# KTH-RPL/cloth-splatting

Hardware: AMD Instinct MI355X
Metric: rasterizer fwd+bwd rendered Mpix/s (scene_1, 800x800) (higher is better)
Workload: dtype f32

## Files before the change

cloth-splatting_amd/csrc/csplat_raster.hip:

```cpp
#include "csplat_common.h"

#include <atomic>
#include <cstring>
#include <chrono>
#include <mutex>
#include <type_traits>

#include "csplat_raster_math.h"
#include "csplat_raster_k1.h"
#include "csplat_raster_binning.h"
#include "csplat_raster_k5b_k6.h"

namespace {

constexpr int ACC_STRIDE = 16;

#define CSPLAT_ROWMASK_OP(OP, dst, src0, src1, RM)                                                                                  \
    asm("s_nop 1\n\tv_" OP "_f32_dpp %0, %1, %2 quad_perm:[0,1,2,3] row_mask:" RM " bank_mask:0xf" : "+v"(dst) : "v"(src0), "v"(src1))
__device__ __forceinline__ void rows_scan_mul(float f, float Tin, float &Tr, float &Tout) {
    const auto s16 = __builtin_amdgcn_permlane16_swap(__float_as_uint(f), __float_as_uint(f), false, false);
    const float ev = __uint_as_float(s16[0]), od = __uint_as_float(s16[1]);
    const float pr = ev * od;
    const auto s32 = __builtin_amdgcn_permlane32_swap(__float_as_uint(pr), __float_as_uint(pr), false, false);
    const float lo = __uint_as_float(s32[0]), hi = __uint_as_float(s32[1]);
// ... 613 lines not shown
    return (g_stamp_buf && g_stamp_words == 8u * ((size_t)cdiv(P, 64) + (size_t)cdiv(P, 32))) ? g_stamp_buf : nullptr;
}

int tsort_mode(int P) { return (P < (1 << 24) ? 1 : 0) | (dbg(CSPLAT_DEBUG_SORT_RADIX_ONLY) ? 2 : 0) | (dbg(CSPLAT_DEBUG_SORT_RADIX_FALLBACK) ? 4 : 0); }

int higher_msb(uint32_t n) {
    int b = 0;
    while ((1u << b) < n && b < 31) b++;
    return b == 0 ? 1 : b;
}

hipEvent_t pooled_event() {
    constexpr int N = 256;
    static hipEvent_t ring[N];
    static std::atomic<unsigned> next{0};
    static std::mutex mu;
    const unsigned k = next.fetch_add(1) % N;
    std::lock_guard<std::mutex> lk(mu);
    if (!ring[k] && hipEventCreateWithFlags(&ring[k], hipEventDisableTiming) != hipSuccess) { (void)hipGetLastError(); return nullptr; }
    return ring[k];
}

}

extern "C" {

int csplat_abi_version(void) { return CSPLAT_ABI_VERSION; }
int csplat_debug_flags(unsigned flags) { g_debug_flags = flags; return 0; }
unsigned csplat_debug_flags_query(void) { return g_debug_flags; }
int csplat_debug_stamps(void *buf, size_t bytes) { g_stamp_buf = (unsigned long long *)buf; g_stamp_words = bytes / 8; return 0; }
}
unsigned long long *csplat_stamp_buffer(size_t need_words) { return (g_stamp_buf && g_stamp_words >= need_words) ? g_stamp_buf : nullptr; }
extern "C" {
const char *csplat_last_error(void) { return g_csplat_err; }

size_t csplat_geom_bytes(int P) { size_t off[G_NFIELDS]; return geom_offsets(P, off); }
size_t csplat_image_bytes(int W, int H) { size_t off[I_NFIELDS]; return image_offsets(W, H, off); }
size_t csplat_binning_bytes(int64_t R, int W, int H) { size_t off[B_NFIELDS]; return binning_offsets(R, tiles_of(W, H), off); }
size_t csplat_temp_bytes(int P, int64_t R, int W, int H) { (void)P; (void)W; (void)H; size_t off[T_NFIELDS]; return temp_offsets(R, off); }
static size_t scratch_bytes(ScratchPath path, int P, int64_t R, int W, int H) {
    size_t off[S_NFIELDS];
    return scratch_offsets(path, P, R, W, H, dbg(CSPLAT_DEBUG_BIT_REPRODUCIBLE), off);
}
size_t csplat_backward_scratch_bytes(int P, int64_t R) { return scratch_bytes(SP_COLOUR, P, R, 0, 0); }
size_t csplat_backward_depth_scratch_bytes(int P, int64_t R, int W, int H) { return scratch_bytes(SP_DEPTH, P, R, W, H); }
size_t csplat_backward_camera_scratch_bytes(int P, int64_t R, int W, int H) { return scratch_bytes(SP_CAMERA, P, R, W, H); }
size_t csplat_backward_feature_scratch_bytes(int P, int64_t R, int W, int H) { return scratch_bytes(SP_FEATURE, P, R, W, H); }
int csplat_geom_layout(int P, size_t *o8) { size_t off[G_NFIELDS]; geom_offsets(P, off); for (int k = 0; k < 8; k++) o8[k] = off[k]; return 0; }
static_assert(B_NFIELDS == 11 && B_KEYS == 0 && B_IDS == 1 && I_RANGES == 0 && I_NCONTRIB == 1 && I_FINALT == 2, "field numbers csplat.h documents");
int csplat_binning_fields(int64_t R, int W, int H, size_t *o11) { binning_offsets(R, tiles_of(W, H), o11); return 0; }
int csplat_binning_layout(int64_t R, int W, int H, size_t *o2) {
    size_t off[B_NFIELDS];
    binning_offsets(R, tiles_of(W, H), off);
    o2[0] = off[B_KEYS]; o2[1] = off[B_IDS];
    return 0;
}
int csplat_image_layout(int W, int H, size_t *o3) {
    size_t off[I_NFIELDS];
    image_offsets(W, H, off);
    o3[0] = off[I_RANGES]; o3[1] = off[I_NCONTRIB]; o3[2] = off[I_FINALT];
    return 0;
}

struct FwdTicket {
    bool used = false;
    hipStream_t s = nullptr;
    int P = 0, W = 0, H = 0, tiles = 0, nb = 0;
    bool can_bucket = false, use_mail = false;
    uint32_t tag = 0;
    volatile uint32_t *mb_host = nullptr;
    Cam cam;
    Geom g;
    void *gbase = nullptr, *ibase = nullptr;
    int2 *ranges = nullptr;
    uint32_t *n_contrib = nullptr, *info = nullptr, *table = nullptr;
    float *final_T = nullptr;
    const float *bg = nullptr;
    int32_t *radii = nullptr;
    csplat_alloc_fn alloc = nullptr;
    void *alloc_ctx = nullptr;
    uint32_t *mb_dev = nullptr;
    int D = 0, M = 0;
    bool aa = false;
    float scale_modifier = 1.f;
    const float *means3D = nullptr, *shs = nullptr, *colors_precomp = nullptr, *opacities = nullptr, *scales = nullptr, *rotations = nullptr,
                *cov3D_precomp = nullptr;
};
constexpr int MAX_TICKETS = 64;
static FwdTicket g_tickets[MAX_TICKETS];
static std::mutex g_ticket_mu;

static int begin_prepare(void *stream, int P, int D, int M, const float *bg, int W, int H, const float *means3D,
                         const float *shs, const float *colors_precomp, const float *opacities, const float *scales,
                         float scale_modifier, const float *rotations, const float *cov3D_precomp, const float *view,
                         const float *proj, const float *campos, float tanfovx, float tanfovy, int prefiltered,
                         csplat_alloc_fn alloc, void *alloc_ctx, int32_t *radii, int *ticket_out) {
    hipStream_t s = (hipStream_t)stream;
    CSPLAT_REQUIRE(P >= 0 && W > 0 && H > 0, "csplat_forward: bad sizes");
    CSPLAT_REQUIRE(ticket_out != nullptr, "csplat_forward_begin: ticket_out missing");
    CSPLAT_REQUIRE(P == 0 || (shs != nullptr) != (colors_precomp != nullptr), "provide exactly one of shs / colors_precomp");
    CSPLAT_REQUIRE(P == 0 || (cov3D_precomp != nullptr) != (scales != nullptr && rotations != nullptr),
                   "provide exactly one of (scales, rotations) / cov3D_precomp");
    CSPLAT_REQUIRE(shs == nullptr || (D >= 0 && D <= 3 && M >= (D + 1) * (D + 1)), "SH degree / coefficient count mismatch");
    CSPLAT_REQUIRE(alloc != nullptr, "allocator callback missing");
    Cam cam;
    make_cam(cam, view, proj, campos, tanfovx, tanfovy, W, H);

    void *gbase = alloc(alloc_ctx, CSPLAT_CHUNK_GEOM, csplat_geom_bytes(P));
    void *ibase = alloc(alloc_ctx, CSPLAT_CHUNK_IMAGE, csplat_image_bytes(W, H));
    CSPLAT_REQUIRE(gbase && ibase, "allocator returned NULL");
    const ImageView im = image_view(ibase, W, H);
    const int tiles = cam.gx * cam.gy;
    const bool can_bucket = tiles <= BUCKET_TILES && !dbg(CSPLAT_DEBUG_GLOBAL_SORT);
    uint32_t *table = nullptr;
    if (can_bucket) {
        table = (uint32_t *)alloc(alloc_ctx, CSPLAT_CHUNK_TABLE, bucket_table_bytes(P, tiles));
        CSPLAT_REQUIRE(table, "allocator returned NULL");
    }
    int tk = -1;
    {
        std::lock_guard<std::mutex> lk(g_ticket_mu);
        for (int i = 0; i < MAX_TICKETS && tk < 0; i++)
            if (!g_tickets[i].used) tk = i;
        if (tk >= 0) g_tickets[tk].used = true;
    }
    CSPLAT_REQUIRE(tk >= 0, "csplat_forward_begin: more than 64 forwards begun and not finished");
    FwdTicket &t = g_tickets[tk];
    t.s = s; t.P = P; t.W = W; t.H = H; t.tiles = tiles; t.nb = cdiv(P > 0 ? P : 1, BUCKET_G); t.can_bucket = can_bucket;
    t.use_mail = false; t.tag = 0; t.mb_host = nullptr; t.mb_dev = nullptr;
    if (can_bucket && !dbg(CSPLAT_DEBUG_NO_MAILBOX) && mail_init()) {
        t.use_mail = true;
        t.tag = g_mail.next.fetch_add(1);
        if (t.tag == 0) t.tag = g_mail.next.fetch_add(1);
        const int slot = (int)(t.tag % MAIL_SLOTS);
        t.mb_host = g_mail.host + slot * MAIL_WORDS;
        t.mb_dev = g_mail.dev + slot * MAIL_WORDS;
    }
    t.cam = cam; t.g = geom_view(gbase, P); t.gbase = gbase; t.ibase = ibase;
    t.ranges = im.ranges; t.n_contrib = im.n_contrib; t.final_T = im.final_T; t.info = im.info;
    t.table = table; t.bg = bg; t.radii = radii; t.alloc = alloc; t.alloc_ctx = alloc_ctx;
    t.D = D; t.M = M; t.means3D = means3D; t.shs = shs; t.colors_precomp = colors_precomp; t.opacities = opacities; t.scales = scales;
    t.scale_modifier = scale_modifier; t.rotations = rotations; t.cov3D_precomp = cov3D_precomp;
    t.aa = (prefiltered & CSPLAT_ANTIALIAS) != 0;
    *ticket_out = tk;
    return 0;
}

static int nocull_mode() { return dbg(CSPLAT_DEBUG_NO_CULLING) ? 1 : dbg(CSPLAT_DEBUG_CULL_RADIUS_X4) ? 2 : 0; }

static int begin_launch(const FwdTicket &t) {
    hipStream_t s = t.s;
    const int P = t.P, tiles = t.tiles, nb = t.nb;
    if (!t.can_bucket) HIP_TRY(hipMemsetAsync(t.ranges, 0, (size_t)tiles * 8, s));
    if (P > 0) {
        ProfScope ps(PROF_K1, s);
        const bool stage = t.shs != nullptr && t.M == 16 && ((uintptr_t)t.shs & 15u) == 0;
        if (t.aa && stage)
            k_preprocess_aa<true><<<cdiv(P, 256), 256, 0, s>>>(P, t.D, t.M, t.means3D, t.shs, t.colors_precomp, t.opacities, t.scales,
                                                                t.scale_modifier, t.rotations, t.cov3D_precomp, t.cam, t.g, t.radii, nocull_mode());
        else if (t.aa)
            k_preprocess_aa<false><<<cdiv(P, 256), 256, 0, s>>>(P, t.D, t.M, t.means3D, t.shs, t.colors_precomp, t.opacities, t.scales,
                                                                 t.scale_modifier, t.rotations, t.cov3D_precomp, t.cam, t.g, t.radii, nocull_mode());
        else if (stage)
            k_preprocess<true><<<cdiv(P, 256), 256, 0, s>>>(P, t.D, t.M, t.means3D, t.shs, t.colors_precomp, t.opacities, t.scales,
                                                             t.scale_modifier, t.rotations, t.cov3D_precomp, t.cam, t.g, t.radii, nocull_mode());
        else
            k_preprocess<false><<<cdiv(P, 256), 256, 0, s>>>(P, t.D, t.M, t.means3D, t.shs, t.colors_precomp, t.opacities, t.scales,
                                                              t.scale_modifier, t.rotations, t.cov3D_precomp, t.cam, t.g, t.radii, nocull_mode());
        LAUNCH_CHECK();
    }
    if (t.can_bucket) {
        ProfScope ps(PROF_K2, s);
        if (P > 0) {
            k_tile_count<<<nb, BUCKET_G, (size_t)tiles * 4, s>>>(P, tiles, t.g.xy, t.radii, t.cam, t.table);
            LAUNCH_CHECK();
        } else {
            HIP_TRY(hipMemsetAsync(t.table, 0, (size_t)nb * tiles * 4, s));
        }
        uint32_t *tile_cnt = t.table + (size_t)nb * tiles;
        k_tile_colscan<<<cdiv(tiles, 256), 256, 0, s>>>(tiles, nb, t.table, tile_cnt);
        LAUNCH_CHECK();
        k_tile_scan<<<1, 1024, 0, s>>>(tiles, tile_cnt, t.ranges, t.info, t.mb_dev, t.tag);
        LAUNCH_CHECK();
    }
    return 0;
}

static bool begin_views_compatible(int V, const int *tk) {
    if (V < 1 || V > RASTER_MAX_VIEWS || dbg(CSPLAT_DEBUG_PER_VIEW_LAUNCHES)) return false;
    const FwdTicket &a = g_tickets[tk[0]];
    if (a.P <= 0 || !a.can_bucket || !a.shs || a.colors_precomp || a.cov3D_precomp || !a.scales || !a.rotations) return false;
    for (int i = 1; i < V; i++) {
        const FwdTicket &w = g_tickets[tk[i]];
        if (w.P != a.P || w.D != a.D || w.M != a.M || w.W != a.W || w.H != a.H || w.shs != a.shs || w.opacities != a.opacities ||
            w.scales != a.scales || w.scale_modifier != a.scale_modifier || w.colors_precomp || w.cov3D_precomp || !w.rotations ||
            !w.can_bucket || w.aa != a.aa)
            return false;
    }
    return true;
}
static int begin_launch_views(int V, const int *tk, hipStream_t join) {
    const FwdTicket &a = g_tickets[tk[0]];
    const int P = a.P, tiles = a.tiles, nb = a.nb;
    K1Table tab;
    tab.n = V;
    for (int i = 0; i < V; i++) {
        const FwdTicket &t = g_tickets[tk[i]];
        K1View &k = tab.v[i];
        k.means3D = t.means3D; k.rotations = t.rotations; k.cam = t.cam; k.g = t.g; k.radii = t.radii; k.table = t.table;
        k.info = t.info; k.mailbox = t.mb_dev; k.ranges = t.ranges; k.tag = t.tag;
    }
    {
        ProfScope ps(PROF_K1, join);
        const bool stage = a.M == 16 && ((uintptr_t)a.shs & 15u) == 0;
        if (a.aa && stage)
            k_preprocess_views_aa<true><<<cdiv(P, K1V_G), 256, 0, join>>>(P, a.D, a.M, a.shs, a.opacities, a.scales, a.scale_modifier, tab,
                                                                        nocull_mode());
        else if (a.aa)
            k_preprocess_views_aa<false><<<cdiv(P, K1V_G), 256, 0, join>>>(P, a.D, a.M, a.shs, a.opacities, a.scales, a.scale_modifier, tab,
                                                                         nocull_mode());
        else if (stage && per_gaussian_stamps(P))
            k_preprocess_views_stamps<<<cdiv(P, K1V_G), 256, 0, join>>>(P, a.D, a.M, a.shs, a.opacities, a.scales, a.scale_modifier, tab,
                                                                      nocull_mode(), per_gaussian_stamps(P));
        else if (stage)
            k_preprocess_views<true><<<cdiv(P, K1V_G), 256, 0, join>>>(P, a.D, a.M, a.shs, a.opacities, a.scales, a.scale_modifier, tab,
                                                                     nocull_mode());
        else
            k_preprocess_views<false><<<cdiv(P, K1V_G), 256, 0, join>>>(P, a.D, a.M, a.shs, a.opacities, a.scales, a.scale_modifier, tab,
                                                                      nocull_mode());
        LAUNCH_CHECK();
    }
    {
        ProfScope ps(PROF_K2, join);
        k_tile_count_views<<<dim3(nb, V), BUCKET_G, (size_t)tiles * 4, join>>>(P, tiles, tab);
        LAUNCH_CHECK();
        k_tile_colscan_views<<<dim3(cdiv(tiles, 256), V), 256, 0, join>>>(tiles, nb, tab);
        LAUNCH_CHECK();
        k_tile_scan_views<<<V, 1024, 0, join>>>(tiles, nb, tab);
        LAUNCH_CHECK();
    }
    return 0;
}

int csplat_forward_begin(void *stream, int P, int D, int M, const float *bg, int W, int H, const float *means3D,
                         const float *shs, const float *colors_precomp, const float *opacities, const float *scales,
                         float scale_modifier, const float *rotations, const float *cov3D_precomp, const float *view,
                         const float *proj, const float *campos, float tanfovx, float tanfovy, int prefiltered,
                         csplat_alloc_fn alloc, void *alloc_ctx, int32_t *radii, int *ticket_out) {
    CSPLAT_REQUIRE(!(prefiltered & CSPLAT_ANTIALIAS), "csplat_forward / csplat_forward_begin: CSPLAT_ANTIALIAS needs a csplat_view entry point "
                                                      "(csplat_forward_views*), whose backward knows the bit");
    if (int rc = begin_prepare(stream, P, D, M, bg, W, H, means3D, shs, colors_precomp, opacities, scales, scale_modifier, rotations,
                               cov3D_precomp, view, proj, campos, tanfovx, tanfovy, prefiltered, alloc, alloc_ctx, radii, ticket_out))
        return rc;
    const int rc = begin_launch(g_tickets[*ticket_out]);
    if (rc) {
        std::lock_guard<std::mutex> lk(g_ticket_mu);
        g_tickets[*ticket_out].used = false;
    }
    return rc;
}

static int finish_read(const FwdTicket &t, uint32_t host_info[3], hipStream_t launched_on = nullptr) {
    hipStream_t s = launched_on ? launched_on : t.s;
    host_info[0] = host_info[1] = host_info[2] = 0;
    if (t.can_bucket) {
        bool got = false;
        if (t.use_mail) {
            const auto t0 = std::chrono::steady_clock::now();
            unsigned spins = 0;
            while (!(got = (t.mb_host[2] == t.tag))) {
                if ((++spins & 0x3FFu) == 0 &&
                    std::chrono::duration<double>(std::chrono::steady_clock::now() - t0).count() > 2.0) break;
            }
            if (got) { host_info[0] = t.mb_host[0]; host_info[1] = t.mb_host[1]; host_info[2] = t.mb_host[3]; }
        }
        if (!got) {
            HIP_TRY(hipMemcpyAsync(host_info, t.info, 12, hipMemcpyDeviceToHost, s));
            HIP_TRY(hipStreamSynchronize(s));
        }
    } else if (t.P > 0) {
        ProfScope ps(PROF_K2, s);
        if (int rc = csplat_inclusive_scan_u32(s, t.g.tiles_touched, t.g.offsets, t.P, t.g.scan_tmp)) return rc;
        HIP_TRY(hipMemcpyAsync(host_info, t.g.offsets + (t.P - 1), 4, hipMemcpyDeviceToHost, s));
        HIP_TRY(hipStreamSynchronize(s));
        host_info[1] = 0xFFFFFFFFu;
        host_info[2] = 0xFFFFFFFFu;
    }
    CSPLAT_REQUIRE(host_info[0] <= 0x7FFFFFFFu, "csplat_forward: more than 2^31 - 1 tile instances (Gaussian x tile pairs) in one view");
    return 0;
}
#define TSORT_FOR_ITEMS(X) X(2) X(4) X(6) X(8)
static int tsort_items(uint32_t longest) {
    const uint32_t items = (longest + TSORT_THREADS - 1) / TSORT_THREADS;
    return items <= 2 ? 2 : items <= 4 ? 4 : items <= 6 ? 6 : 8;
}
static bool tsort_dense(int items, uint64_t busy) {
    static int s_cus = 0;
    if (s_cus <= 0) {
        int dev = 0;
        if (hipGetDevice(&dev) != hipSuccess || hipDeviceGetAttribute(&s_cus, hipDeviceAttributeMultiprocessorCount, dev) != hipSuccess || s_cus <= 0)
            s_cus = 256;
        (void)hipGetLastError();
    }
    return items <= 6 && 2 * busy > 5 * (uint64_t)s_cus;
}
static uint32_t tile_sort_cap() {
    static int s_lds_big = -1;
    if (s_lds_big < 0) {
        bool ok = true;
#define X(I) ok = ok && hipFuncSetAttribute((const void *)k_tile_sort<I, false>, hipFuncAttributeMaxDynamicSharedMemorySize, 96 * 1024) == hipSuccess && \
                  hipFuncSetAttribute((const void *)k_tile_sort<I, I <= 6>, hipFuncAttributeMaxDynamicSharedMemorySize, 96 * 1024) == hipSuccess &&  \
                  hipFuncSetAttribute((const void *)k_tile_sort_views<I, false>, hipFuncAttributeMaxDynamicSharedMemorySize, 96 * 1024) == hipSuccess && \
                  hipFuncSetAttribute((const void *)k_tile_sort_views<I, I <= 6>, hipFuncAttributeMaxDynamicSharedMemorySize, 96 * 1024) == hipSuccess;
        TSORT_FOR_ITEMS(X)
#undef X
        s_lds_big = ok;
        (void)hipGetLastError();
    }
    return s_lds_big ? (uint32_t)BUCKET_CAP : 5120u;
}
static void tile_sort_launch(hipStream_t s, int tiles, uint32_t longest, uint32_t busy, const int2 *ranges, const uint64_t *comp,
                             uint64_t *keys_sorted, uint32_t *ids_sorted, const uint32_t *info, int mode) {
    const size_t lds = tsort_lds_bytes((int)longest);
    const int grid = tiles < TSORT_GRID ? tiles : TSORT_GRID, items = tsort_items(longest);
    const bool dense = tsort_dense(items, busy);
    switch (items) {
#define X(I) case I:                                                                                                                        \
        if (dense) k_tile_sort<I, I <= 6><<<grid, TSORT_THREADS, lds, s>>>(ranges, comp, keys_sorted, ids_sorted, info, tiles, mode);       \
        else k_tile_sort<I, false><<<grid, TSORT_THREADS, lds, s>>>(ranges, comp, keys_sorted, ids_sorted, info, tiles, mode);              \
        break;
        TSORT_FOR_ITEMS(X)
#undef X
    }
}
static void tile_sort_views_launch(hipStream_t s, int tiles, int V, uint32_t Lcap, uint32_t Bcap, const P2Table &tab, int mode) {
    const size_t lds = tsort_lds_bytes((int)Lcap);
    const dim3 grid(tiles < TSORT_GRID ? tiles : TSORT_GRID, V);
    const int items = tsort_items(Lcap);
    const bool dense = tsort_dense(items, (uint64_t)V * (Bcap < (uint32_t)tiles ? Bcap : (uint32_t)tiles));
    switch (items) {
#define X(I) case I:                                                                                           \
        if (dense) k_tile_sort_views<I, I <= 6><<<grid, TSORT_THREADS, lds, s>>>(tab, tiles, mode);            \
        else k_tile_sort_views<I, false><<<grid, TSORT_THREADS, lds, s>>>(tab, tiles, mode);                   \
        break;
        TSORT_FOR_ITEMS(X)
#undef X
    }
}

struct SpecHist { int W = 0, H = 0, P = 0; uint32_t R = 0, longest = 0, busy = 0; };
constexpr int SPEC_RING = 8;
static SpecHist g_spec_ring[SPEC_RING];
static int g_spec_next = 0;
static std::mutex g_spec_mu;

struct PendingViews {
    bool used = false;
    const csplat_view *key = nullptr;
    int V = 0, tk[RASTER_MAX_VIEWS];
    uint32_t Rcap[RASTER_MAX_VIEWS], Lcap = 0, Bcap = 0;
};
constexpr int MAX_PENDING = 8;
static PendingViews g_pending[MAX_PENDING];
static std::mutex g_pending_mu;

static int p2_launch(int V, const int *tk, csplat_view *v, hipStream_t join, const uint32_t *Rcap, uint32_t Lcap, int spec, uint32_t Bcap,
                     uint32_t *valid = nullptr) {
    const FwdTicket &a = g_tickets[tk[0]];
    const int P = a.P, W = a.W, H = a.H, tiles = a.tiles, nb = a.nb;
    {
        P2Table tab;
        tab.valid = valid; tab.nviews = V;
        uint32_t maxR = 0;
        for (int i = 0; i < V; i++) {
            const FwdTicket &t = g_tickets[tk[i]];
            const uint32_t R = Rcap[i];
            maxR = R > maxR ? R : maxR;
            void *bbase = t.alloc(t.alloc_ctx, CSPLAT_CHUNK_BINNING, csplat_binning_bytes(R, W, H));
            void *tbase = t.alloc(t.alloc_ctx, CSPLAT_CHUNK_TEMP, csplat_temp_bytes(P, R, W, H));
            CSPLAT_REQUIRE(bbase && tbase, "allocator returned NULL");
            const BinView b = binning_view(bbase, R, tiles);
            P2View &k = tab.v[i];
            k.g = t.g; k.cam = t.cam; k.radii = t.radii; k.table = t.table; k.ranges = t.ranges;
            k.keys_u = temp_view(tbase, R).keys_u;
            k.keys_sorted = b.keys_sorted; k.ids_sorted = b.ids_sorted; k.seg_offset = b.seg_offset; k.slot_tile = b.slot_tile;
            k.ckpt = b.ckpt; k.mask16 = b.mask16; k.bbits = b.bbits; k.bmask = b.bmask; k.recA = b.recA; k.recB = b.recB; k.recC = b.recC;
            k.bg = t.bg; k.final_T = t.final_T; k.n_contrib = t.n_contrib; k.out_color = v[i].out_color; k.out_depth = v[i].out_depth;
            k.R = R; k.info = t.info; k.Lcap = Lcap; k.Bcap = Bcap; k.spec = spec;
            v[i].layout_rendered = (int)R; v[i].geom = t.gbase; v[i].binning = bbase; v[i].image = t.ibase;
// ... 1017 lines not shown
```

cloth-splatting_amd/csrc/csplat_raster_binning.h:

```cpp
#pragma once

namespace {

__global__ __launch_bounds__(256) void k_emit_keys(int P, const float2 *__restrict__ xy, const float *__restrict__ depth,
                                                    const uint32_t *__restrict__ offsets,
                                                    const int32_t *__restrict__ radii, Cam cam,
                                                    uint64_t *__restrict__ keys, uint32_t *__restrict__ ids) {
    const int i = blockIdx.x * blockDim.x + threadIdx.x;
    if (i >= P) return;
    const int rad = radii[i];
    if (rad <= 0) return;
    uint32_t off = (i == 0) ? 0u : offsets[i - 1];
    const float2 p = xy[i];
    int minx, miny, maxx, maxy;
    tile_rect(p.x, p.y, rad, cam, minx, miny, maxx, maxy);
    const uint32_t dbits = __float_as_uint(depth[i]);
    for (int y = miny; y < maxy; y++)
        for (int x = minx; x < maxx; x++) {
            keys[off] = ((uint64_t)(uint32_t)(y * cam.gx + x) << 32) | dbits;
            ids[off] = (uint32_t)i;
            off++;
        }
}

__global__ __launch_bounds__(256) void k_tile_ranges(int64_t R, const uint64_t *__restrict__ keys, int2 *__restrict__ ranges) {
    const int64_t i = (int64_t)blockIdx.x * blockDim.x + threadIdx.x;
    if (i >= R) return;
    const uint32_t t = (uint32_t)(keys[i] >> 32);
    if (i == 0) ranges[t].x = 0;
    else {
        const uint32_t tp = (uint32_t)(keys[i - 1] >> 32);
        if (tp != t) { ranges[tp].y = (int)i; ranges[t].x = (int)i; }
    }
    if (i == R - 1) ranges[t].y = (int)R;
}

constexpr int BUCKET_CAP = 8192;
constexpr int BUCKET_TILES = 12288;
constexpr int BUCKET_G = 1024;

__device__ __forceinline__ void tile_count_body(int P, int tiles, const float2 *__restrict__ xy,
                                                const int32_t *__restrict__ radii, const Cam &cam,
                                                uint32_t *__restrict__ table) {
    extern __shared__ uint32_t s_hist[];
    for (int t = threadIdx.x; t < tiles; t += BUCKET_G) s_hist[t] = 0u;
    __syncthreads();
    const int i = blockIdx.x * BUCKET_G + threadIdx.x;
    if (i < P) {
        const int rad = radii[i];
        if (rad > 0) {
            const float2 p = xy[i];
            int minx, miny, maxx, maxy;
            tile_rect(p.x, p.y, rad, cam, minx, miny, maxx, maxy);
            for (int y = miny; y < maxy; y++)
                for (int x = minx; x < maxx; x++) atomicAdd(&s_hist[y * cam.gx + x], 1u);
        }
    }
    __syncthreads();
    uint32_t *row = table + (size_t)blockIdx.x * tiles;
    for (int t = threadIdx.x; t < tiles; t += BUCKET_G) row[t] = s_hist[t];
}
__global__ __launch_bounds__(BUCKET_G) void k_tile_count(int P, int tiles, const float2 *__restrict__ xy,
                                                          const int32_t *__restrict__ radii, Cam cam,
                                                          uint32_t *__restrict__ table) {
    tile_count_body(P, tiles, xy, radii, cam, table);
}
__global__ __launch_bounds__(BUCKET_G) void k_tile_count_views(int P, int tiles, K1Table tab) {
    const K1View &w = tab.v[blockIdx.y];
    tile_count_body(P, tiles, w.g.xy, w.radii, w.cam, w.table);
}

__device__ __forceinline__ void tile_colscan_body(int tiles, int nb, uint32_t *__restrict__ table, uint32_t *__restrict__ cnt) {
    const int t = blockIdx.x * 256 + threadIdx.x;
    if (t >= tiles) return;
    uint32_t run = 0;
    int b = 0;
    for (; b + 8 <= nb; b += 8) {
        uint32_t v[8];
#pragma unroll
        for (int u = 0; u < 8; u++) v[u] = table[(size_t)(b + u) * tiles + t];
#pragma unroll
        for (int u = 0; u < 8; u++) { table[(size_t)(b + u) * tiles + t] = run; run += v[u]; }
    }
    for (; b < nb; b++) { const uint32_t v = table[(size_t)b * tiles + t]; table[(size_t)b * tiles + t] = run; run += v; }
    cnt[t] = run;
}
__global__ __launch_bounds__(256) void k_tile_colscan(int tiles, int nb, uint32_t *__restrict__ table, uint32_t *__restrict__ cnt) {
    tile_colscan_body(tiles, nb, table, cnt);
}
__global__ __launch_bounds__(256) void k_tile_colscan_views(int tiles, int nb, K1Table tab) {
    uint32_t *table = tab.v[blockIdx.y].table;
    tile_colscan_body(tiles, nb, table, table + (size_t)nb * tiles);
}

constexpr int INFO_BUSY = 64;
constexpr int LPT_BINS = 512;
constexpr int TSCAN_ITEMS = BUCKET_TILES / 1024;
__device__ __forceinline__ void tile_scan_body(int tiles, const uint32_t *__restrict__ cnt, int2 *__restrict__ ranges,
                                               uint32_t *__restrict__ info, volatile uint32_t *mailbox, uint32_t tag) {
    __shared__ unsigned long long s_w[17];
    __shared__ uint32_t s_max[16];
    __shared__ uint32_t s_bin[LPT_BINS + 1];
    const int lane = threadIdx.x & 63, w = threadIdx.x >> 6;
    uint32_t *busy = info + INFO_BUSY;
    uint32_t *lpt = busy + tiles + 4;
    const int per = (tiles + 1023) / 1024, t0 = threadIdx.x * per;
    uint32_t c[TSCAN_ITEMS];
#pragma unroll
    for (int k = 0; k < TSCAN_ITEMS; k++) c[k] = (k < per && t0 + k < tiles) ? cnt[t0 + k] : 0u;
    for (int i = threadIdx.x; i <= LPT_BINS; i += 1024) s_bin[i] = 0u;
    uint32_t mx = 0;
    unsigned long long v0 = 0ull;
#pragma unroll
    for (int k = 0; k < TSCAN_ITEMS; k++) { mx = max(mx, c[k]); v0 += (unsigned long long)c[k] | ((unsigned long long)(c[k] ? 1u : 0u) << 32); }
    unsigned long long inc = v0;
#pragma unroll
    for (int d = 1; d < 64; d <<= 1) { const unsigned long long o = __shfl_up(inc, d, 64); if (lane >= d) inc += o; }
    if (lane == 63) s_w[w] = inc;
    __syncthreads();
    if (w == 0) {
        unsigned long long v = lane < 16 ? s_w[lane] : 0ull, vi = v;
#pragma unroll
        for (int d = 1; d < 16; d <<= 1) { const unsigned long long o = __shfl_up(vi, d, 64); if (lane >= d) vi += o; }
        if (lane < 16) s_w[lane] = vi - v;
        if (lane == 15) s_w[16] = vi;
    }
    __syncthreads();
    const unsigned long long carry = s_w[16];
    {
        unsigned long long exl = s_w[w] + inc - v0;
#pragma unroll
        for (int k = 0; k < TSCAN_ITEMS; k++) {
            const int t = t0 + k;
            if (k < per && t < tiles) {
                const uint32_t ex = (uint32_t)exl, nz = (uint32_t)(exl >> 32);
                ranges[t] = c[k] ? make_int2((int)ex, (int)(ex + c[k])) : make_int2(0, 0);
                if (c[k]) {
                    busy[1 + nz] = (uint32_t)t;
                    atomicAdd(&s_bin[LPT_BINS - 1 - min(c[k] >> 4, (uint32_t)(LPT_BINS - 1))], 1u);
                } else {
                    lpt[tiles - 1 - (t - (int)nz)] = (uint32_t)t;
                }
                exl += (unsigned long long)c[k] | ((unsigned long long)(c[k] ? 1u : 0u) << 32);
            }
        }
    }
    __syncthreads();
    {
        if (w == 0) {
            uint32_t v[LPT_BINS / 64], run = 0;
#pragma unroll
            for (int k = 0; k < LPT_BINS / 64; k++) { v[k] = s_bin[lane * (LPT_BINS / 64) + k]; run += v[k]; }
            uint32_t binc = run;
#pragma unroll
            for (int d = 1; d < 64; d <<= 1) { const uint32_t o = (uint32_t)__shfl_up((int)binc, d, 64); if (lane >= d) binc += o; }
            uint32_t base = binc - run;
#pragma unroll
            for (int k = 0; k < LPT_BINS / 64; k++) { s_bin[lane * (LPT_BINS / 64) + k] = base; base += v[k]; }
        }
        __syncthreads();
#pragma unroll
        for (int k = 0; k < TSCAN_ITEMS; k++)
            if (c[k]) lpt[atomicAdd(&s_bin[LPT_BINS - 1 - min(c[k] >> 4, (uint32_t)(LPT_BINS - 1))], 1u)] = (uint32_t)(t0 + k);
    }
#pragma unroll
    for (int d = 32; d > 0; d >>= 1) mx = max(mx, (uint32_t)__shfl_xor((int)mx, d, 64));
    if (lane == 0) s_max[w] = mx;
    __syncthreads();
    if (threadIdx.x == 0) {
        uint32_t m = 0;
        for (int k = 0; k < 16; k++) m = max(m, s_max[k]);
        info[0] = (uint32_t)carry;
        info[1] = m;
        info[2] = (uint32_t)(carry >> 32);
        busy[0] = (uint32_t)(carry >> 32);
        if (mailbox) {
            mailbox[0] = (uint32_t)carry;
            mailbox[1] = m;
            mailbox[3] = (uint32_t)(carry >> 32);
            __threadfence_system();
            mailbox[2] = tag;
        }
    }
}
__global__ __launch_bounds__(1024) void k_tile_scan(int tiles, const uint32_t *__restrict__ cnt, int2 *__restrict__ ranges,
                                                     uint32_t *__restrict__ info, volatile uint32_t *mailbox, uint32_t tag) {
    tile_scan_body(tiles, cnt, ranges, info, mailbox, tag);
}
__global__ __launch_bounds__(1024) void k_tile_scan_views(int tiles, int nb, K1Table tab) {
    const K1View &w = tab.v[blockIdx.x];
    tile_scan_body(tiles, w.table + (size_t)nb * tiles, w.ranges, w.info, w.mailbox, w.tag);
}

__device__ __forceinline__ void emit_bucket_body(int P, int tiles, const float2 *__restrict__ xy,
                                                 const float *__restrict__ depth, const int32_t *__restrict__ radii,
                                                 const Cam &cam, const uint32_t *__restrict__ table,
                                                 const int2 *__restrict__ ranges, uint64_t *__restrict__ comp) {
    extern __shared__ uint32_t s_base[];
    const uint32_t *row = table + (size_t)blockIdx.x * tiles;
    for (int t = threadIdx.x; t < tiles; t += BUCKET_G) s_base[t] = (uint32_t)ranges[t].x + row[t];
    __syncthreads();
    const int i = blockIdx.x * BUCKET_G + threadIdx.x;
    if (i >= P) return;
    const int rad = radii[i];
    if (rad <= 0) return;
    const float2 p = xy[i];
    int minx, miny, maxx, maxy;
    tile_rect(p.x, p.y, rad, cam, minx, miny, maxx, maxy);
    const uint64_t v = ((uint64_t)__float_as_uint(depth[i]) << 32) | (uint32_t)i;
    for (int y = miny; y < maxy; y++)
        for (int x = minx; x < maxx; x++) comp[atomicAdd(&s_base[y * cam.gx + x], 1u)] = v;
}
__global__ __launch_bounds__(BUCKET_G) void k_emit_bucket(int P, int tiles, const float2 *__restrict__ xy,
                                                           const float *__restrict__ depth, const int32_t *__restrict__ radii,
                                                           Cam cam, const uint32_t *__restrict__ table,
                                                           const int2 *__restrict__ ranges, uint64_t *__restrict__ comp) {
    emit_bucket_body(P, tiles, xy, depth, radii, cam, table, ranges, comp);
}

struct P2View {
    Geom g;
    Cam cam;
    const int32_t *radii;
    const uint32_t *table;
    int2 *ranges;
    uint64_t *keys_u, *keys_sorted;
    uint32_t *ids_sorted;
    int *seg_offset, *slot_tile;
    float4 *ckpt;
    uint16_t *mask16;
    unsigned long long *bbits;
    unsigned long long *bmask;
    float4 *recA, *recB;
    float2 *recC;
    const float *bg;
    float *final_T;
    uint32_t *n_contrib;
    float *out_color, *out_depth;
    uint32_t R;
    const uint32_t *info;
    uint32_t Lcap;
    uint32_t Bcap;
    int spec;
};
struct P2Table { P2View v[RASTER_MAX_VIEWS]; uint32_t *valid; int nviews; };
// ... 372 lines not shown
```

cloth-splatting_amd/csrc/csplat_raster_k1.h:

```cpp
#pragma once

namespace {

struct K1In {
    float p[3];
    float sq[7];
    float op;
};
__device__ __forceinline__ void k1_request(int P, const float *__restrict__ means3D, const float *__restrict__ opacities,
                                           const float *__restrict__ scales, const float *__restrict__ rotations,
                                           const float *__restrict__ cov3D_precomp, int i, K1In &in) {
    const int il = min(i, P - 1);
#pragma unroll
    for (int k = 0; k < 3; k++) in.p[k] = means3D[3 * il + k];
    if (cov3D_precomp) {
#pragma unroll
        for (int k = 0; k < 6; k++) in.sq[k] = cov3D_precomp[6 * il + k];
        in.sq[6] = 0.f;
    } else {
#pragma unroll
        for (int k = 0; k < 3; k++) in.sq[k] = scales[3 * il + k];
#pragma unroll
        for (int k = 0; k < 4; k++) in.sq[3 + k] = rotations[4 * il + k];
    }
    in.op = opacities[il];
}

template <int NT, int ROWS>
__device__ __forceinline__ void stage_sh_rows_batched(const float *__restrict__ src, int rows, float *s_rows) {
    constexpr int N = (ROWS * 12 + NT - 1) / NT;
    const float4 *src4 = reinterpret_cast<const float4 *>(src);
    const int n = rows * 12;
    float4 v[N];
#pragma unroll
    for (int k = 0; k < N; k++) v[k] = src4[min((int)threadIdx.x + k * NT, n - 1)];
#pragma unroll
    for (int k = 0; k < N; k++) {
        const int t = (int)threadIdx.x + k * NT;
        if (t < n) {
            const int row = t / 12, c = (t - row * 12) * 4;
            float *d = s_rows + row * SH_ROW + c;
            d[0] = v[k].x; d[1] = v[k].y; d[2] = v[k].z; d[3] = v[k].w;
        }
    }
}

struct NoMark {
    __device__ __forceinline__ void operator()(int, float) const {}
};
struct StampMark {
    unsigned long long *at;
    __device__ __forceinline__ void operator()(int k, float dep) const {
        if (threadIdx.x == 0) {
            asm volatile("" ::"v"(dep) : "memory");
            at[k] = (unsigned long long)__builtin_amdgcn_s_memtime();
            asm volatile("" ::: "memory");
        }
    }
};

template <bool STAGE, bool AA = false, class MK = NoMark>
__device__ __forceinline__ void preprocess_body(int P, int D, int M, const K1In &in, const float *__restrict__ shs,
                                                const float *__restrict__ colors_precomp, float scale_mod, bool cov_precomp,
                                                const Cam &cam, const Geom &g, int32_t *__restrict__ radii, int nocull,
                                                const float *s_shrows, int i, int srow, const MK &mark = MK()) {
#pragma clang fp contract(off)
    if (i >= P) return;
    float depth = 0.f, px = 0.f, py = 0.f, cut = -1.f;
    float4 co = {0.f, 0.f, 0.f, 0.f};
    float rgb[3] = {0.f, 0.f, 0.f};
    float c6[6] = {0.f, 0.f, 0.f, 0.f, 0.f, 0.f};
    uint32_t clampbits = 0, touched = 0;
    int rad = 0;

    const float p[3] = {in.p[0], in.p[1], in.p[2]};
    mark(2, p[2]);
    float pv[3];
    view_point(p, cam.view, pv);
    do {
        if (pv[2] <= NEAR_Z) break;
        const float *pr = cam.proj;
        const float hx = pr[0] * p[0] + pr[4] * p[1] + pr[8] * p[2] + pr[12];
        const float hy = pr[1] * p[0] + pr[5] * p[1] + pr[9] * p[2] + pr[13];
        const float hw = pr[3] * p[0] + pr[7] * p[1] + pr[11] * p[2] + pr[15];
        const float pw = 1.0f / (hw + 0.0000001f);
        const float ndcx = hx * pw, ndcy = hy * pw;
        if (cov_precomp) {
#pragma unroll
            for (int k = 0; k < 6; k++) c6[k] = in.sq[k];
        } else {
            const float s[3] = {in.sq[0], in.sq[1], in.sq[2]};
            const float q[4] = {in.sq[3], in.sq[4], in.sq[5], in.sq[6]};
            mark(3, q[3]);
            cov3d_from_scale_rot(s, scale_mod, q, c6);
        }
        ProjJac pj;
        proj_jacobian(pv, cam, pj);
        float a, b, c;
        float aa_h = 1.f;
        if constexpr (AA) {
            float a0, c0;
            cov2d_undilated(c6, pj, a0, b, c0);
            a = a0 + AA_DILATE; c = c0 + AA_DILATE;
            aa_h = aa_factor(a0, b, c0);
        } else {
            cov2d_from_cov3d(c6, pj, a, b, c);
        }
        const float det = a * c - b * b;
        if (det == 0.0f) break;
        const float det_inv = 1.f / det;
        const float mid = 0.5f * (a + c);
        const float sq = sqrtf(fmaxf(0.1f, mid * mid - det));
        const float lam1 = mid + sq, lam2 = mid - sq;
        const float my_radius = ceilf(3.f * sqrtf(fmaxf(lam1, lam2)));
        const float ix = ((ndcx + 1.0f) * (float)cam.W - 1.0f) * 0.5f;
        const float iy = ((ndcy + 1.0f) * (float)cam.H - 1.0f) * 0.5f;
        const int r = (int)my_radius;
        int minx, miny, maxx, maxy;
        tile_rect(ix, iy, r, cam, minx, miny, maxx, maxy);
        if ((maxx - minx) * (maxy - miny) == 0) break;

        if (colors_precomp) {
#pragma unroll
            for (int k = 0; k < 3; k++) rgb[k] = colors_precomp[3 * i + k];
        } else {
            const float *sh = STAGE ? (const float *)(s_shrows + srow * SH_ROW) : shs + (size_t)i * M * 3;
            const float d0 = p[0] - cam.campos[0], d1 = p[1] - cam.campos[1], d2 = p[2] - cam.campos[2];
            const float len = sqrtf(d0 * d0 + d1 * d1 + d2 * d2);
            const float x = d0 / len, y = d1 / len, z = d2 / len;
#pragma unroll
            for (int ch = 0; ch < 3; ch++) {
#define S(k) sh[(k) * 3 + ch]
                float res = SH_C0 * S(0);
                if (D > 0) {
                    res = res - SH_C1 * y * S(1) + SH_C1 * z * S(2) - SH_C1 * x * S(3);
                    if (D > 1) {
                        const float xx = x * x, yy = y * y, zz = z * z, xy = x * y, yz = y * z, xz = x * z;
                        res = res + SH_C2[0] * xy * S(4) + SH_C2[1] * yz * S(5) + SH_C2[2] * (2.f * zz - xx - yy) * S(6) +
                              SH_C2[3] * xz * S(7) + SH_C2[4] * (xx - yy) * S(8);
                        if (D > 2) {
                            res = res + SH_C3[0] * y * (3.f * xx - yy) * S(9) + SH_C3[1] * xy * z * S(10) +
                                  SH_C3[2] * y * (4.f * zz - xx - yy) * S(11) +
                                  SH_C3[3] * z * (2.f * zz - 3.f * xx - 3.f * yy) * S(12) +
                                  SH_C3[4] * x * (4.f * zz - xx - yy) * S(13) + SH_C3[5] * z * (xx - yy) * S(14) +
                                  SH_C3[6] * x * (xx - 3.f * yy) * S(15);
                        }
                    }
                }
#undef S
                res += 0.5f;
                if (res < 0.f) clampbits |= (1u << ch);
                rgb[ch] = fmaxf(res, 0.f);
            }
        }
        depth = pv[2];
        rad = r;
        px = ix; py = iy;
        float op = in.op;
        mark(4, op);
        if constexpr (AA) op = op * aa_h;
        co = make_float4(c * det_inv, -b * det_inv, a * det_inv, op);
        touched = (uint32_t)((maxy - miny) * (maxx - minx));
        const float cancel = 4e-7f * (a * c + b * b) / det;
        cut = cancel < 0.25f ? 2.f * lam1 * logf(255.f * op) * (1.0001f + 2.f * cancel) + 0.01f : 3.0e38f;
        if (nocull == 1) cut = 3.0e38f;
        if (nocull == 2) cut = cut * 4.f + 4.f;
    } while (0);

    g.depth[i] = depth;
    radii[i] = rad;
    g.xy[i] = make_float2(px, py);
    g.conic_opacity[i] = co;
#pragma unroll
    for (int k = 0; k < 3; k++) g.rgb[3 * i + k] = rgb[k];
#pragma unroll
    for (int k = 0; k < 6; k++) g.cov3D[6 * i + k] = c6[k];
    g.clamped[i] = clampbits;
    g.tiles_touched[i] = touched;
    g.cut2[i] = cut;
    g.pack[3 * (size_t)i] = make_float4(px, py, co.x, co.y);
    g.pack[3 * (size_t)i + 1] = make_float4(co.z, co.w, rgb[0], rgb[1]);
    g.pack[3 * (size_t)i + 2] = make_float4(rgb[2], depth, cut, 0.f);
    mark(5, 0.f);
}

template <bool STAGE>
__global__ __launch_bounds__(256) void k_preprocess(int P, int D, int M, const float *__restrict__ means3D,
                                                     const float *__restrict__ shs,
                                                     const float *__restrict__ colors_precomp,
                                                     const float *__restrict__ opacities,
                                                     const float *__restrict__ scales, float scale_mod,
                                                     const float *__restrict__ rotations,
                                                     const float *__restrict__ cov3D_precomp, Cam cam, Geom g,
                                                     int32_t *__restrict__ radii, int nocull) {
    __shared__ float s_shrows[STAGE ? 256 * SH_ROW : 1];
    const int i = (int)(blockIdx.x * blockDim.x + threadIdx.x);
    K1In in;
    k1_request(P, means3D, opacities, scales, rotations, cov3D_precomp, i, in);
    if (STAGE) {
        const int base = blockIdx.x * 256;
        stage_sh_rows<256>(shs + (size_t)base * 48, min(256, P - base), s_shrows);
        __syncthreads();
    }
    preprocess_body<STAGE>(P, D, M, in, shs, colors_precomp, scale_mod, cov3D_precomp != nullptr, cam, g, radii, nocull, s_shrows, i,
                           (int)threadIdx.x);
}
template <bool STAGE>
__global__ __launch_bounds__(256) void k_preprocess_aa(int P, int D, int M, const float *__restrict__ means3D,
                                                        const float *__restrict__ shs,
                                                        const float *__restrict__ colors_precomp,
                                                        const float *__restrict__ opacities,
                                                        const float *__restrict__ scales, float scale_mod,
                                                        const float *__restrict__ rotations,
                                                        const float *__restrict__ cov3D_precomp, Cam cam, Geom g,
                                                        int32_t *__restrict__ radii, int nocull) {
    __shared__ float s_shrows[STAGE ? 256 * SH_ROW : 1];
    const int i = (int)(blockIdx.x * blockDim.x + threadIdx.x);
    K1In in;
    k1_request(P, means3D, opacities, scales, rotations, cov3D_precomp, i, in);
    if (STAGE) {
        const int base = blockIdx.x * 256;
        stage_sh_rows<256>(shs + (size_t)base * 48, min(256, P - base), s_shrows);
        __syncthreads();
    }
    preprocess_body<STAGE, true>(P, D, M, in, shs, colors_precomp, scale_mod, cov3D_precomp != nullptr, cam, g, radii, nocull, s_shrows, i,
                                 (int)threadIdx.x);
}

struct K1View {
    const float *means3D, *rotations;
    Cam cam;
    Geom g;
    int32_t *radii;
    uint32_t *table, *info, *mailbox;
    int2 *ranges;
    uint32_t tag;
};
struct K1Table { int n; K1View v[RASTER_MAX_VIEWS]; };

constexpr int K1V_G = 64;
template <bool STAGE, bool AA, class MK>
__device__ __forceinline__ void preprocess_views(int P, int D, int M, const float *__restrict__ shs, const float *__restrict__ opacities,
                                                 const float *__restrict__ scales, float scale_mod, const K1Table &tab, int nocull,
                                                 float *s_shrows, const MK &mark) {
    mark(0, 0.f);
    const int base = blockIdx.x * K1V_G;
    const int lane = threadIdx.x & 63;
    if (tab.n <= 0) return;
    const int wave = __builtin_amdgcn_readfirstlane((int)(threadIdx.x >> 6));
    K1In in;
    {
        const K1View &w0 = tab.v[min(wave, tab.n - 1)];
        k1_request(P, w0.means3D, opacities, scales, w0.rotations, nullptr, base + lane, in);
    }
    if (STAGE) {
        stage_sh_rows_batched<256, K1V_G>(shs + (size_t)base * 48, min(K1V_G, P - base), s_shrows);
        __syncthreads();
    }
    mark(1, 0.f);
    for (int vi = wave; vi < tab.n; vi += 4) {
        const K1View &w = tab.v[vi];
        preprocess_body<STAGE, AA>(P, D, M, in, shs, nullptr, scale_mod, false, w.cam, w.g, w.radii, nocull, s_shrows, base + lane, lane, mark);
        if (vi + 4 < tab.n) k1_request(P, tab.v[vi + 4].means3D, opacities, scales, tab.v[vi + 4].rotations, nullptr, base + lane, in);
    }
}
template <bool STAGE>
__global__ __launch_bounds__(256) void k_preprocess_views(int P, int D, int M, const float *__restrict__ shs,
                                                           const float *__restrict__ opacities,
                                                           const float *__restrict__ scales, float scale_mod, K1Table tab,
                                                           int nocull) {
    __shared__ float s_shrows[STAGE ? K1V_G * SH_ROW : 1];
    preprocess_views<STAGE, false>(P, D, M, shs, opacities, scales, scale_mod, tab, nocull, s_shrows, NoMark());
}
template <bool STAGE>
__global__ __launch_bounds__(256) void k_preprocess_views_aa(int P, int D, int M, const float *__restrict__ shs,
                                                              const float *__restrict__ opacities,
                                                              const float *__restrict__ scales, float scale_mod, K1Table tab,
                                                              int nocull) {
    __shared__ float s_shrows[STAGE ? K1V_G * SH_ROW : 1];
    preprocess_views<STAGE, true>(P, D, M, shs, opacities, scales, scale_mod, tab, nocull, s_shrows, NoMark());
}
__global__ __launch_bounds__(256) void k_preprocess_views_stamps(int P, int D, int M, const float *__restrict__ shs,
                                                                  const float *__restrict__ opacities,
                                                                  const float *__restrict__ scales, float scale_mod, K1Table tab,
                                                                  int nocull, unsigned long long *stamp_buf) {
    __shared__ float s_shrows[K1V_G * SH_ROW];
    preprocess_views<true, false>(P, D, M, shs, opacities, scales, scale_mod, tab, nocull, s_shrows, StampMark{stamp_buf + (size_t)blockIdx.x * 8});
}

}
```

Measured before the change: 4849.

## Replace per-tile column scan kernel with atomic offset allocation in tile count

Removes the separate column-scan kernel that turned per-block tile histograms into prefix offsets. Each block of the tile-count kernel now atomically adds its histogram into a per-tile total and stores the returned value as its base offset. The totals are zeroed inside the preprocess kernel. This saves a launch and a full pass over the nb×tiles table. In exchange, block order within a tile is no longer deterministic, so the order of Gaussians within a tile may vary between runs, and the tile-count kernel now issues global atomics.

After: 4839. Within noise of the previous version (-0.2%).

```diff
diff --git a/cloth-splatting_amd/csrc/csplat_raster.hip b/cloth-splatting_amd/csrc/csplat_raster.hip
--- a/cloth-splatting_amd/csrc/csplat_raster.hip
+++ b/cloth-splatting_amd/csrc/csplat_raster.hip
@@ -789,21 +789,22 @@
     hipStream_t s = t.s;
     const int P = t.P, tiles = t.tiles, nb = t.nb;
     if (!t.can_bucket) HIP_TRY(hipMemsetAsync(t.ranges, 0, (size_t)tiles * 8, s));
+    uint32_t *tile_cnt = t.can_bucket ? t.table + (size_t)nb * tiles : nullptr;
     if (P > 0) {
         ProfScope ps(PROF_K1, s);
         const bool stage = t.shs != nullptr && t.M == 16 && ((uintptr_t)t.shs & 15u) == 0;
         if (t.aa && stage)
             k_preprocess_aa<true><<<cdiv(P, 256), 256, 0, s>>>(P, t.D, t.M, t.means3D, t.shs, t.colors_precomp, t.opacities, t.scales,
-                                                                t.scale_modifier, t.rotations, t.cov3D_precomp, t.cam, t.g, t.radii, nocull_mode());
+                                                                t.scale_modifier, t.rotations, t.cov3D_precomp, t.cam, t.g, t.radii, nocull_mode(), tile_cnt);
         else if (t.aa)
             k_preprocess_aa<false><<<cdiv(P, 256), 256, 0, s>>>(P, t.D, t.M, t.means3D, t.shs, t.colors_precomp, t.opacities, t.scales,
-                                                                 t.scale_modifier, t.rotations, t.cov3D_precomp, t.cam, t.g, t.radii, nocull_mode());
+                                                                 t.scale_modifier, t.rotations, t.cov3D_precomp, t.cam, t.g, t.radii, nocull_mode(), tile_cnt);
         else if (stage)
             k_preprocess<true><<<cdiv(P, 256), 256, 0, s>>>(P, t.D, t.M, t.means3D, t.shs, t.colors_precomp, t.opacities, t.scales,
-                                                             t.scale_modifier, t.rotations, t.cov3D_precomp, t.cam, t.g, t.radii, nocull_mode());
+                                                             t.scale_modifier, t.rotations, t.cov3D_precomp, t.cam, t.g, t.radii, nocull_mode(), tile_cnt);
         else
             k_preprocess<false><<<cdiv(P, 256), 256, 0, s>>>(P, t.D, t.M, t.means3D, t.shs, t.colors_precomp, t.opacities, t.scales,
-                                                              t.scale_modifier, t.rotations, t.cov3D_precomp, t.cam, t.g, t.radii, nocull_mode());
+                                                              t.scale_modifier, t.rotations, t.cov3D_precomp, t.cam, t.g, t.radii, nocull_mode(), tile_cnt);
         LAUNCH_CHECK();
     }
     if (t.can_bucket) {
@@ -812,11 +813,8 @@
             k_tile_count<<<nb, BUCKET_G, (size_t)tiles * 4, s>>>(P, tiles, t.g.xy, t.radii, t.cam, t.table);
             LAUNCH_CHECK();
         } else {
-            HIP_TRY(hipMemsetAsync(t.table, 0, (size_t)nb * tiles * 4, s));
-        }
-        uint32_t *tile_cnt = t.table + (size_t)nb * tiles;
-        k_tile_colscan<<<cdiv(tiles, 256), 256, 0, s>>>(tiles, nb, t.table, tile_cnt);
-        LAUNCH_CHECK();
+            HIP_TRY(hipMemsetAsync(t.table, 0, (size_t)(nb + 1) * tiles * 4, s));
+        }
         k_tile_scan<<<1, 1024, 0, s>>>(tiles, tile_cnt, t.ranges, t.info, t.mb_dev, t.tag);
         LAUNCH_CHECK();
     }
@@ -870,8 +868,6 @@
     {
         ProfScope ps(PROF_K2, join);
         k_tile_count_views<<<dim3(nb, V), BUCKET_G, (size_t)tiles * 4, join>>>(P, tiles, tab);
-        LAUNCH_CHECK();
-        k_tile_colscan_views<<<dim3(cdiv(tiles, 256), V), 256, 0, join>>>(tiles, nb, tab);
         LAUNCH_CHECK();
         k_tile_scan_views<<<V, 1024, 0, join>>>(tiles, nb, tab);
         LAUNCH_CHECK();
diff --git a/cloth-splatting_amd/csrc/csplat_raster_binning.h b/cloth-splatting_amd/csrc/csplat_raster_binning.h
--- a/cloth-splatting_amd/csrc/csplat_raster_binning.h
+++ b/cloth-splatting_amd/csrc/csplat_raster_binning.h
@@ -37,7 +37,6 @@
 
 constexpr int BUCKET_CAP = 8192;
 constexpr int BUCKET_TILES = 12288;
-constexpr int BUCKET_G = 1024;
 
 __device__ __forceinline__ void tile_count_body(int P, int tiles, const float2 *__restrict__ xy,
                                                 const int32_t *__restrict__ radii, const Cam &cam,
@@ -58,7 +57,17 @@
     }
     __syncthreads();
     uint32_t *row = table + (size_t)blockIdx.x * tiles;
-    for (int t = threadIdx.x; t < tiles; t += BUCKET_G) row[t] = s_hist[t];
+    uint32_t *cnt = table + (size_t)gridDim.x * tiles;
+    for (int t0 = threadIdx.x; t0 < tiles; t0 += 4 * BUCKET_G) {
+        uint32_t h[4], b[4];
+#pragma unroll
+        for (int u = 0; u < 4; u++) { const int t = t0 + u * BUCKET_G; h[u] = t < tiles ? s_hist[t] : 0u; }
+#pragma unroll
+        for (int u = 0; u < 4; u++)
+            b[u] = h[u] ? __hip_atomic_fetch_add(&cnt[t0 + u * BUCKET_G], h[u], __ATOMIC_RELAXED, __HIP_MEMORY_SCOPE_AGENT) : 0u;
+#pragma unroll
+        for (int u = 0; u < 4; u++) { const int t = t0 + u * BUCKET_G; if (t < tiles) row[t] = b[u]; }
+    }
 }
 __global__ __launch_bounds__(BUCKET_G) void k_tile_count(int P, int tiles, const float2 *__restrict__ xy,
                                                           const int32_t *__restrict__ radii, Cam cam,
@@ -68,29 +77,6 @@
 __global__ __launch_bounds__(BUCKET_G) void k_tile_count_views(int P, int tiles, K1Table tab) {
     const K1View &w = tab.v[blockIdx.y];
     tile_count_body(P, tiles, w.g.xy, w.radii, w.cam, w.table);
-}
-
-__device__ __forceinline__ void tile_colscan_body(int tiles, int nb, uint32_t *__restrict__ table, uint32_t *__restrict__ cnt) {
-    const int t = blockIdx.x * 256 + threadIdx.x;
-    if (t >= tiles) return;
-    uint32_t run = 0;
-    int b = 0;
-    for (; b + 8 <= nb; b += 8) {
-        uint32_t v[8];
-#pragma unroll
-        for (int u = 0; u < 8; u++) v[u] = table[(size_t)(b + u) * tiles + t];
-#pragma unroll
-        for (int u = 0; u < 8; u++) { table[(size_t)(b + u) * tiles + t] = run; run += v[u]; }
-    }
-    for (; b < nb; b++) { const uint32_t v = table[(size_t)b * tiles + t]; table[(size_t)b * tiles + t] = run; run += v; }
-    cnt[t] = run;
-}
-__global__ __launch_bounds__(256) void k_tile_colscan(int tiles, int nb, uint32_t *__restrict__ table, uint32_t *__restrict__ cnt) {
-    tile_colscan_body(tiles, nb, table, cnt);
-}
-__global__ __launch_bounds__(256) void k_tile_colscan_views(int tiles, int nb, K1Table tab) {
-    uint32_t *table = tab.v[blockIdx.y].table;
-    tile_colscan_body(tiles, nb, table, table + (size_t)nb * tiles);
 }
 
 constexpr int INFO_BUSY = 64;
diff --git a/cloth-splatting_amd/csrc/csplat_raster_k1.h b/cloth-splatting_amd/csrc/csplat_raster_k1.h
--- a/cloth-splatting_amd/csrc/csplat_raster_k1.h
+++ b/cloth-splatting_amd/csrc/csplat_raster_k1.h
@@ -24,6 +24,11 @@
         for (int k = 0; k < 4; k++) in.sq[3 + k] = rotations[4 * il + k];
     }
     in.op = opacities[il];
+}
+
+constexpr int BUCKET_G = 1024;
+__device__ __forceinline__ void k1_clear_counts(uint32_t *__restrict__ cnt, int tiles) {
+    for (int t = (int)(blockIdx.x * 256 + threadIdx.x); t < tiles; t += (int)(gridDim.x * 256)) cnt[t] = 0u;
 }
 
 template <int NT, int ROWS>
@@ -192,11 +197,12 @@
                                                      const float *__restrict__ scales, float scale_mod,
                                                      const float *__restrict__ rotations,
                                                      const float *__restrict__ cov3D_precomp, Cam cam, Geom g,
-                                                     int32_t *__restrict__ radii, int nocull) {
+                                                     int32_t *__restrict__ radii, int nocull, uint32_t *__restrict__ tile_cnt) {
     __shared__ float s_shrows[STAGE ? 256 * SH_ROW : 1];
     const int i = (int)(blockIdx.x * blockDim.x + threadIdx.x);
     K1In in;
     k1_request(P, means3D, opacities, scales, rotations, cov3D_precomp, i, in);
+    if (tile_cnt) k1_clear_counts(tile_cnt, cam.gx * cam.gy);
     if (STAGE) {
         const int base = blockIdx.x * 256;
         stage_sh_rows<256>(shs + (size_t)base * 48, min(256, P - base), s_shrows);
@@ -213,11 +219,12 @@
                                                         const float *__restrict__ scales, float scale_mod,
                                                         const float *__restrict__ rotations,
                                                         const float *__restrict__ cov3D_precomp, Cam cam, Geom g,
-                                                        int32_t *__restrict__ radii, int nocull) {
+                                                        int32_t *__restrict__ radii, int nocull, uint32_t *__restrict__ tile_cnt) {
     __shared__ float s_shrows[STAGE ? 256 * SH_ROW : 1];
     const int i = (int)(blockIdx.x * blockDim.x + threadIdx.x);
     K1In in;
     k1_request(P, means3D, opacities, scales, rotations, cov3D_precomp, i, in);
+    if (tile_cnt) k1_clear_counts(tile_cnt, cam.gx * cam.gy);
     if (STAGE) {
         const int base = blockIdx.x * 256;
         stage_sh_rows<256>(shs + (size_t)base * 48, min(256, P - base), s_shrows);
@@ -253,6 +260,11 @@
         const K1View &w0 = tab.v[min(wave, tab.n - 1)];
         k1_request(P, w0.means3D, opacities, scales, w0.rotations, nullptr, base + lane, in);
     }
+    {
+        const int tiles = tab.v[0].cam.gx * tab.v[0].cam.gy;
+        if ((int)(blockIdx.x * 256) < tiles)
+            for (int vi = 0; vi < tab.n; vi++) k1_clear_counts(tab.v[vi].table + (size_t)((P + BUCKET_G - 1) / BUCKET_G) * tiles, tiles);
+    }
     if (STAGE) {
         stage_sh_rows_batched<256, K1V_G>(shs + (size_t)base * 48, min(K1V_G, P - base), s_shrows);
         __syncthreads();
```
